# cindytsai/multigrid_poisson_solver

Hardware: AMD Instinct MI355X
Metric: vcycle_mlups (higher is better)
Workload: dtype f64; 1 GPU; V(3,3)-cycle N=8192^2 fp64, 11 levels to N=8, red-black GS(1e-7) coarse solve, cycle-file driver (eager, stream smoother: temporally blocked wave-streaming kernels on the large levels, register-tile kernels on the levels 65..1024, one-workgroup LDS kernel below; halos recomputed, neighbours via DPP lane shifts); N=8192, levels=11

## Files before the change

### include/mg_hip.h

```cpp
#ifndef MG_HIP_H
#define MG_HIP_H

#include <stddef.h>
#include <stdint.h>

#ifdef __cplusplus
extern "C" {
#endif

int         mg_init(int device);
void        mg_finalize(void);
void        mg_set_stream(void *hip_stream);
void       *mg_get_stream(void);
void        mg_sync(void);
int         mg_last_error(void);
const char *mg_last_error_string(void);
void        mg_clear_error(void);
void        mg_set_abort_on_error(int on);
int         mg_set_smoother(const char *name);
const char *mg_version(void);

double *mg_alloc(size_t n_doubles);
void    mg_free(double *dev);
void    mg_pool_trim(void);
// ... 36 lines not shown
void   mg_download_f32(float *host, const float *dev, size_t n);
void mg_prolongAdd(int N, const double *U_c, int M, const double *U_f_in, double *U_f_out);
void mg_restrict_signed(int N, const double *U_f, int M, double *U_c, int sign);
int  mg_lastExactSolverIterations(void);

void mg_restriction_table(int N, int M, int *lo, double *w);
void mg_prolongation_table(int N, int M, int axis, int *owner, double *w_hi, double *w_lo);

void mg_fill_uniform(double *dst, size_t n_doubles, uint64_t seed);
void mg_checksum(const double *src, size_t n_doubles, uint64_t out[2]);

typedef struct mg_profile_entry {
    char   name[64];
    int    N;
    int    launches;
    double total_ms;
    double algo_bytes;
} mg_profile_entry;
void mg_profile_begin(int min_N);
void mg_profile_sample(int every);
int  mg_profile_end(mg_profile_entry *out, int cap);

typedef struct mg_node_record {
    int    node;
    int    N;
    int    steps;
    double error;
} mg_node_record;

typedef struct mg_cycle_result {
    int     status;
    int     N;
    double *U_dev;
    double  mg_error;
    double  time_ms;
    double  device_ms;
    int     n_records;
    const mg_node_record *records;
    const char *report;
    int     graph_replayed;
    int     schedule_launches;
} mg_cycle_result;

typedef struct mg_cycle_plan mg_cycle_plan;

#define MG_CYCLE_FUSED   1
#define MG_CYCLE_GRAPH   2
#define MG_CYCLE_REPORT  4
#define MG_CYCLE_ERROR   8
#define MG_CYCLE_MIXED  16

mg_cycle_plan *mg_cycle_load(const char *path, int flags);
int            mg_cycle_execute(mg_cycle_plan *plan, mg_cycle_result *out);
int            mg_cycle_enqueue(mg_cycle_plan *plan);
int            mg_cycle_collect(mg_cycle_plan *plan, mg_cycle_result *out);
int            mg_cycle_set_refinement(mg_cycle_plan *plan, int cycles);
int            mg_cycle_refinement_errors(mg_cycle_plan *plan, double *out, int cap);
void           mg_cycle_destroy(mg_cycle_plan *plan);
int            mg_cycle_main(int argc, char **argv);
int            mg_print2File(int N, const double *U_dev, const char *file_name);

int  mg_comm_unique_id_bytes(void);
int  mg_comm_get_unique_id(void *out);
int  mg_comm_init(int rank, int nranks, const void *unique_id);
typedef struct mg_host_transport {
    void *user;
    int (*exchange)(void *user, int n_ops, const int *is_send, const int *peer, void *const *buf, const size_t *bytes);
    int (*allgather)(void *user, const double *send, double *recv, size_t count_per_rank);
} mg_host_transport;
int  mg_comm_init_host(int rank, int nranks, const mg_host_transport *transport);
int  mg_comm_selftest(size_t n_doubles);
void mg_comm_finalize(void);
int  mg_comm_rank(void);
int  mg_comm_size(void);
const char *mg_comm_library(void);

int  mg_slab_partition(int N_max, int N_min, int nranks, int collapse_N, int *out, int *collapsed_out);
int  mg_slab_ghost_rows(void);
int  mg_slab_schedule(int N_max, int N_min, int nranks, int collapse_N, int steps, int ca_mode, int ca_pct,
                      int *level_out, int *rank_out);
int  mg_slab_recompute_levels(int N_max, int N_min, int steps, int *pre_out);
int  mg_slab_recompute_levels_ranks(int N_max, int N_min, int steps, int nranks, int *pre_out);
int  mg_recompute_pair_available(int pre, int post);

typedef struct mg_slab_plan mg_slab_plan;
mg_slab_plan *mg_slab_load(const char *path, int nranks, int rank, int collapse_N);
mg_slab_plan *mg_slab_load_flags(const char *path, int nranks, int rank, int collapse_N, int flags);
int  mg_slab_set_refinement(mg_slab_plan *plan, int cycles);
int  mg_slab_refinement_errors(mg_slab_plan *plan, double *out, int cap);
int  mg_slab_execute(mg_slab_plan *plan, mg_cycle_result *out);
int  mg_slab_enqueue(mg_slab_plan *plan);
int  mg_slab_collect(mg_slab_plan *plan, mg_cycle_result *out);
int  mg_slab_gather_U(mg_slab_plan *plan, double *host_full);
void mg_slab_want_error(mg_slab_plan *plan, int on);
void mg_slab_destroy(mg_slab_plan *plan);

typedef struct mg_solve_opts {
    int    pre, post;
    int    N_min;
    double omega;
    double coarse_rtol, coarse_atol;
    int    coarse_max_iters;
    double rtol, atol;
    int    max_cycles;
    double shift;
} mg_solve_opts;

#define MG_SOLVE_CONVERGED      0
#define MG_SOLVE_NOT_CONVERGED (-1)

typedef struct mg_solve_result {
    int    status;
    int    cycles;
    int    converged;
    int    coarse_capped;
    double res0, res, ref_norm;
    double device_ms;
    int    n_history;
    const double *history;
} mg_solve_result;

typedef struct mg_solver mg_solver;

void       mg_solve_opts_default(mg_solve_opts *o);
mg_solver *mg_solver_create(int N, double L, const mg_solve_opts *o);
int        mg_solver_solve(mg_solver *s, const double *F_dev, double *U_dev, mg_solve_result *out);
void       mg_solver_destroy(mg_solver *s);

typedef struct mg_batch_solve_stats {
    int    cycles;
    int    launches;
    double device_ms;
} mg_batch_solve_stats;

typedef struct mg_batch_solver mg_batch_solver;

mg_batch_solver *mg_batch_solver_create(int N, double L, int max_batch, const mg_solve_opts *o);
int  mg_batch_solver_solve(mg_batch_solver *s, int n, const double *const *F_dev, double *const *U_dev, mg_solve_result *out,
                           mg_batch_solve_stats *stats);
void mg_batch_solver_destroy(mg_batch_solver *s);

#ifdef __cplusplus
}
#endif
#endif
```

### multigrid_poisson_solver_amd/__init__.py

```python
import ctypes as C
import importlib.util
import os
import sys

import numpy as np

_PKG = os.path.dirname(os.path.abspath(__file__))
LIB_PATH = os.environ.get("MG_LIB") or os.path.join(_PKG, "lib", "libmgpoisson.so")
EXE_PATH = os.path.join(_PKG, "bin", "MG_HIP")

MG_CYCLE_FUSED, MG_CYCLE_GRAPH, MG_CYCLE_REPORT, MG_CYCLE_ERROR, MG_CYCLE_MIXED = 1, 2, 4, 8, 16


class MGError(RuntimeError):
    pass


class NodeRecord(C.Structure):
    _fields_ = [("node", C.c_int), ("N", C.c_int), ("steps", C.c_int), ("error", C.c_double)]


class ProfileEntry(C.Structure):
    _fields_ = [("name", C.c_char * 64), ("N", C.c_int), ("launches", C.c_int), ("total_ms", C.c_double),
                ("algo_bytes", C.c_double)]


class CycleResult(C.Structure):
    _fields_ = [("status", C.c_int), ("N", C.c_int), ("U_dev", C.c_void_p), ("mg_error", C.c_double),
                ("time_ms", C.c_double), ("device_ms", C.c_double), ("n_records", C.c_int),
                ("records", C.POINTER(NodeRecord)), ("report", C.c_char_p), ("graph_replayed", C.c_int),
                ("schedule_launches", C.c_int)]


_vp, _i, _d, _sz, _u64 = C.c_void_p, C.c_int, C.c_double, C.c_size_t, C.c_uint64
_dptr = C.POINTER(C.c_double)


class SolveOpts(C.Structure):
    _fields_ = [("pre", C.c_int), ("post", C.c_int), ("N_min", C.c_int), ("omega", C.c_double), ("coarse_rtol", C.c_double),
                ("coarse_atol", C.c_double), ("coarse_max_iters", C.c_int), ("rtol", C.c_double), ("atol", C.c_double),
                ("max_cycles", C.c_int), ("shift", C.c_double)]


class SolveResult(C.Structure):
    _fields_ = [("status", C.c_int), ("cycles", C.c_int), ("converged", C.c_int), ("coarse_capped", C.c_int),
                ("res0", C.c_double), ("res", C.c_double), ("ref_norm", C.c_double), ("device_ms", C.c_double),
                ("n_history", C.c_int), ("history", _dptr)]


class BatchSolveStats(C.Structure):
    _fields_ = [("cycles", C.c_int), ("launches", C.c_int), ("device_ms", C.c_double)]


MG_SOLVE_CONVERGED, MG_SOLVE_NOT_CONVERGED = 0, -1

ABI = {
    "mg_init": (_i, [_i]), "mg_finalize": (None, []), "mg_set_stream": (None, [_vp]),
    "mg_get_stream": (_vp, []), "mg_sync": (None, []), "mg_last_error": (_i, []),
    "mg_last_error_string": (C.c_char_p, []), "mg_clear_error": (None, []),
    "mg_set_abort_on_error": (None, [_i]), "mg_set_smoother": (_i, [C.c_char_p]),
    "mg_version": (C.c_char_p, []), "mg_set_source": (_i, [C.c_char_p]), "mg_source_mode": (C.c_char_p, []),
    "mg_source_is_bit_identical": (_i, []),
    "mg_alloc": (_vp, [_sz]), "mg_free": (None, [_vp]), "mg_pool_trim": (None, []),
    "mg_pool_bytes": (_sz, []), "mg_upload": (None, [_vp, _vp, _sz]), "mg_download": (None, [_vp, _vp, _sz]),
    "mg_copy": (None, [_vp, _vp, _sz]), "mg_fill_zero": (None, [_vp, _sz]), "mg_negate": (None, [_i, _vp]),
    "mg_getSource": (None, [_i, _d, _vp, _d, _d]), "mg_getAnalytic": (None, [_i, _d, _vp, _d, _d]),
    "mg_analyticError": (None, [_i, _d, _vp, _d, _d, _dptr]),
    "mg_getResidual": (None, [_i, _d, _vp, _vp, _vp]), "mg_doGridAddition": (None, [_i, _vp, _vp]),
    "mg_doSmoothing": (None, [_i, _d, _vp, _vp, _i, _dptr]),
    "mg_doExactSolver": (None, [_i, _d, _vp, _vp, _d, _i]),
    "mg_doRestriction": (None, [_i, _vp, _i, _vp]), "mg_doProlongation": (None, [_i, _vp, _i, _vp]),
    "mg_smooth_pp": (None, [_i, _d, _vp, _vp, _vp, _i, _vp, _vp, _i]),
    "mg_smooth_restrict": (None, [_i, _d, _vp, _vp, _vp, _i, _vp, _i, _vp]),
    "mg_prolong_smooth": (None, [_i, _vp, _i, _d, _vp, _vp, _vp, _i, _vp]),
    "mg_cycle_set_refinement": (_i, [_vp, _i]), "mg_cycle_refinement_errors": (_i, [_vp, _vp, _i]),
    "mg_smooth_restrict_f32": (None, [_i, _d, _vp, _vp, _vp, _i, _vp, _i, _vp]),
    "mg_prolong_smooth_f32": (None, [_i, _vp, _i, _d, _vp, _vp, _vp, _i, _vp]),
    "mg_alloc_f32": (_vp, [_sz]), "mg_free_f32": (None, [_vp]), "mg_to_f32": (None, [_vp, _vp, _sz]),
    "mg_to_f64": (None, [_vp, _vp, _sz]), "mg_upload_f32": (None, [_vp, _vp, _sz]),
    "mg_download_f32": (None, [_vp, _vp, _sz]),
    "mg_prolongAdd": (None, [_i, _vp, _i, _vp, _vp]), "mg_restrict_signed": (None, [_i, _vp, _i, _vp, _i]),
    "mg_lastExactSolverIterations": (_i, []),
    "mg_restriction_table": (None, [_i, _i, _vp, _vp]),
    "mg_prolongation_table": (None, [_i, _i, _i, _vp, _vp, _vp]),
    "mg_fill_uniform": (None, [_vp, _sz, _u64]), "mg_checksum": (None, [_vp, _sz, C.POINTER(_u64)]),
    "mg_cycle_load": (_vp, [C.c_char_p, _i]), "mg_cycle_execute": (_i, [_vp, C.POINTER(CycleResult)]),
    "mg_cycle_enqueue": (_i, [_vp]), "mg_cycle_collect": (_i, [_vp, C.POINTER(CycleResult)]),
    "mg_cycle_destroy": (None, [_vp]), "mg_cycle_main": (_i, [_i, C.POINTER(C.c_char_p)]),
    "mg_print2File": (_i, [_i, _vp, C.c_char_p]),
    "mg_comm_unique_id_bytes": (_i, []), "mg_comm_get_unique_id": (_i, [_vp]),
    "mg_comm_init_host": (_i, [_i, _i, _vp]),
    "mg_comm_init": (_i, [_i, _i, _vp]), "mg_comm_finalize": (None, []), "mg_comm_selftest": (_i, [_sz]), "mg_comm_rank": (_i, []),
    "mg_comm_size": (_i, []),
    "mg_comm_library": (C.c_char_p, []),
    "mg_slab_partition": (_i, [_i, _i, _i, _i, _vp, _vp]), "mg_slab_ghost_rows": (_i, []),
    "mg_slab_set_refinement": (_i, [_vp, _i]), "mg_slab_refinement_errors": (_i, [_vp, _vp, _i]),
    "mg_slab_schedule": (_i, [_i, _i, _i, _i, _i, _i, _i, _vp, _vp]),
    "mg_slab_recompute_levels": (_i, [_i, _i, _i, _vp]), "mg_slab_recompute_levels_ranks": (_i, [_i, _i, _i, _i, _vp]),
    "mg_recompute_pair_available": (_i, [_i, _i]),
    "mg_slab_load": (_vp, [C.c_char_p, _i, _i, _i]), "mg_slab_load_flags": (_vp, [C.c_char_p, _i, _i, _i, _i]), "mg_slab_execute": (_i, [_vp, C.POINTER(CycleResult)]),
    "mg_slab_enqueue": (_i, [_vp]), "mg_slab_collect": (_i, [_vp, C.POINTER(CycleResult)]),
    "mg_slab_gather_U": (_i, [_vp, _vp]), "mg_slab_want_error": (None, [_vp, _i]), "mg_slab_destroy": (None, [_vp]),
    "mg_solve_opts_default": (None, [C.POINTER(SolveOpts)]),
    "mg_solver_create": (_vp, [_i, _d, C.POINTER(SolveOpts)]),
    "mg_solver_solve": (_i, [_vp, _vp, _vp, C.POINTER(SolveResult)]), "mg_solver_destroy": (None, [_vp]),
    "mg_batch_solver_create": (_vp, [_i, _d, _i, C.POINTER(SolveOpts)]),
    "mg_batch_solver_solve": (_i, [_vp, _i, _vp, _vp, _vp, C.POINTER(BatchSolveStats)]),
    "mg_batch_solver_destroy": (None, [_vp]),
    "mg_profile_begin": (None, [_i]), "mg_profile_sample": (None, [_i]), "mg_profile_end": (_i, [C.POINTER(ProfileEntry), _i]),
}

_lib = None
hip_runtime = None


def _bind_hip_runtime():
    global hip_runtime
    mode = os.environ.get("MG_HIP_RUNTIME", "auto")
    hip_runtime = "system"
    if mode == "system":
        return
    if mode not in ("auto", "torch"):
        C.CDLL(mode, mode=C.RTLD_GLOBAL)
        hip_runtime = mode
        return
    if "torch" in sys.modules:
        hip_runtime = "torch (imported before the engine)"
        return
    try:
        spec = importlib.util.find_spec("torch")
    except (ImportError, ValueError):
        spec = None
    if spec is None or not spec.submodule_search_locations:
        return
    cand = os.path.join(list(spec.submodule_search_locations)[0], "lib", "libamdhip64.so")
    if os.path.exists(cand):
        C.CDLL(cand, mode=C.RTLD_GLOBAL)
        hip_runtime = cand


def load_library(path=None):
    global _lib
    if _lib is not None:
        return _lib
    path = path or LIB_PATH
    if not os.path.exists(path):
        raise MGError(f"{path} is missing: run `python -c 'import __graft_entry__ as g; g.build()'` "
                      "(hipcc, gfx950).  There is no CPU fallback.")
    _bind_hip_runtime()
    lib = C.CDLL(path, mode=C.RTLD_GLOBAL)
    missing = []
    for name, (res, args) in ABI.items():
        try:
            fn = getattr(lib, name)
        except AttributeError:
            missing.append(name)
            continue
        fn.restype, fn.argtypes = res, args
    if missing:
        raise MGError(f"{path} does not export: {missing}")
    _lib = lib
    return lib


def _check():
    code = _lib.mg_last_error()
    if code:
        msg = _lib.mg_last_error_string().decode()
        _lib.mg_clear_error()
        raise MGError(f"[{code}] {msg}")


_initialised = False


def init(device=0):
    global _initialised
    lib = load_library()
    lib.mg_set_abort_on_error(0)
    if lib.mg_init(int(device)) != 0:
        code = lib.mg_last_error()
        msg = lib.mg_last_error_string().decode()
# ... 799 lines not shown
```

### multigrid_poisson_solver_amd/csrc/mg_abi.cpp

```cpp
#include <cmath>
#include <cstdarg>
#include <cstdlib>
#include <cstring>

#include "mg_internal.h"

namespace mg {

Context &ctx()
{
    static Context c;
    return c;
}

void fail(int code, const char *fmt, ...)
{
    char buf[512];
    va_list ap;
    va_start(ap, fmt);
    vsnprintf(buf, sizeof buf, fmt, ap);
    va_end(ap);
    Context &c = ctx();
    c.last_error = code;
    c.last_error_text = buf;
    fprintf(stderr, "[ ERROR ]: %s\n", buf);
    if (c.abort_on_error) exit(1);
}

bool hip_ok(hipError_t e, const char *what, const char *file, int line)
{
    if (e == hipSuccess) return true;
    fail(MG_ERR_HIP, "HIP call failed: %s -> %s (%s:%d)", what, hipGetErrorString(e), file, line);
    return false;
}

bool require_ready(const char *who)
{
    if (ctx().ready) return true;
    fail(MG_ERR_NOT_INIT, "%s: mg_init() has not been called (or failed); there is no CPU fallback", who);
    return false;
}

void *Pool::get(size_t bytes)
{
    if (bytes == 0) bytes = 8;
    bytes = (bytes + 255) & ~(size_t)255;
    auto it = free_.find(bytes);
    if (it != free_.end()) {
        void *p = it->second;
        free_.erase(it);
        live_[p] = bytes;
        if (poison_) poison_block(p, bytes);
        return p;
    }
    void *p = nullptr;
    hipError_t e = hipMalloc(&p, bytes);
    if (e != hipSuccess) {
        (void)hipGetLastError();
        trim();
        if (!MG_HIP(hipMalloc(&p, bytes))) return nullptr;
    }
    held_ += bytes;
    live_[p] = bytes;
    if (poison_) poison_block(p, bytes);
    return p;
}

bool pool_poison_wanted()
{
    const char *e = getenv("MG_POOL_POISON");
    return e && strcmp(e, "0") != 0;
}

void poison_block(void *p, size_t bytes)
{
    if (!p) return;
    hipStream_t s = ctx().stream;
    hipStreamCaptureStatus cs = hipStreamCaptureStatusNone;
    if (hipStreamIsCapturing(s, &cs) != hipSuccess) (void)hipGetLastError();
    if (cs != hipStreamCaptureStatusNone) return;
    (void)MG_HIP(hipMemsetAsync(p, 0xFF, bytes, s));
}

void Pool::put(void *p)
{
    if (!p) return;
    auto it = live_.find(p);
    if (it == live_.end()) {
// ... 1012 lines not shown
}

void mg_restrict_signed(int N, const double *U_f, int M, double *U_c, int sign)
{
    if (!require_ready("doRestriction") || !grid_args_ok("doRestriction", N) || !grid_args_ok("doRestriction", M)) return;
    const RestrictTable &t = restrict_table(N, M);
    if (!t.lo) return;
    ProfScope ps("restrict", N, 8.0 * N * N + 8.0 * M * M);
    k::restrict_gather(ctx().stream, N, U_f, M, U_c, t, sign < 0 ? -1 : +1);
}

void mg_doRestriction(int N, double *U_f, int M, double *U_c) { mg_restrict_signed(N, U_f, M, U_c, +1); }

void mg_doProlongation(int N, double *U_c, int M, double *U_f)
{
    if (!require_ready("doProlongation") || !grid_args_ok("doProlongation", N) || !grid_args_ok("doProlongation", M)) return;
    const ProlongTable &t = prolong_table(N, M);
    if (!t.owner_row) return;
    ProfScope ps("prolong", M, 8.0 * N * N + 8.0 * M * M);
    k::prolong(ctx().stream, N, U_c, M, nullptr, U_f, t);
}

void mg_prolongAdd(int N, const double *U_c, int M, const double *U_f_in, double *U_f_out)
{
    if (!require_ready("mg_prolongAdd") || !grid_args_ok("mg_prolongAdd", N) || !grid_args_ok("mg_prolongAdd", M)) return;
    const ProlongTable &t = prolong_table(N, M);
    if (!t.owner_row) return;
    ProfScope ps("prolong_add", M, 8.0 * N * N + 16.0 * M * M);
    k::prolong(ctx().stream, N, U_c, M, U_f_in, U_f_out, t);
}

void mg_profile_begin(int min_N)
{
    if (!require_ready("mg_profile_begin")) return;
    Context &c = ctx();
    (void)hipStreamSynchronize(c.stream);
    for (auto &r : c.prof) {
        c.event_pool.push_back(r.e0);
        c.event_pool.push_back(r.e1);
    }
    c.prof.clear();
    c.profile_min_N = min_N;
    c.profile_window = 0;
    c.profiling = true;
}

void mg_profile_sample(int every) { ctx().profile_every = every < 1 ? 1 : every; }

int mg_profile_end(mg_profile_entry *out, int cap)
{
    if (!require_ready("mg_profile_end")) return 0;
    Context &c = ctx();
    c.profiling = false;
    (void)hipStreamSynchronize(c.stream);
    int count = 0;
    for (auto &r : c.prof) {
        float ms = 0.f;
        if (hipEventElapsedTime(&ms, r.e0, r.e1) != hipSuccess) {
            (void)hipGetLastError();
            ms = 0.f;
        }
        int j = 0;
        for (; j < count; ++j)
            if (out[j].N == r.N && r.name == out[j].name) break;
        if (j == count) {
            if (count >= cap) continue;
            memset(&out[j], 0, sizeof out[j]);
            snprintf(out[j].name, sizeof out[j].name, "%s", r.name.c_str());
            out[j].N = r.N;
            out[j].algo_bytes = r.bytes;
            ++count;
        }
        out[j].launches += 1;
        out[j].total_ms += ms;
        c.event_pool.push_back(r.e0);
        c.event_pool.push_back(r.e1);
    }
    c.prof.clear();
    return count;
}

int mg_recompute_pair_available(int pre, int post) { return k::stream_recompute_supported(pre, post) ? 1 : 0; }

void mg_restriction_table(int N, int M, int *lo, double *w) { build_restriction_table(N, M, lo, w); }
void mg_prolongation_table(int N, int M, int axis, int *owner, double *w_hi, double *w_lo)
{
    build_prolongation_table(N, M, axis, owner, w_hi, w_lo);
}

void mg_fill_uniform(double *dst, size_t n, uint64_t seed)
{
    if (!require_ready("mg_fill_uniform")) return;
    k::fill_uniform(ctx().stream, dst, n, seed);
}

void mg_checksum(const double *src, size_t n, uint64_t out[2])
{
    if (!require_ready("mg_checksum")) return;
    Context &c = ctx();
    uint64_t *slot = (uint64_t *)(c.scalars + Scalars::CHECKSUM);
    k::checksum(c.stream, src, n, slot);
    if (MG_HIP(hipMemcpyAsync(c.host_scalars, slot, 2 * sizeof(uint64_t), hipMemcpyDeviceToHost, c.stream)) &&
        MG_HIP(hipStreamSynchronize(c.stream))) {
        memcpy(out, c.host_scalars, 2 * sizeof(uint64_t));
    }
}

}
```

### multigrid_poisson_solver_amd/csrc/mg_stream_impl.h

```cpp
#include <hip/hip_runtime.h>

#include <type_traits>
#include <utility>

#include <algorithm>
#include <cstdlib>
#include <vector>

#include "mg_divconst.h"
#include "mg_internal.h"
#include "mg_lane_ops.h"

#if !defined(MG_REAL) || !defined(MG_REAL_NS)
#error "define MG_REAL (double|float) and MG_REAL_NS (f64|f32) before including mg_stream_impl.h"
#endif

namespace mg {
namespace k {
namespace MG_REAL_NS {

typedef MG_REAL real_t;

constexpr int PF_DEFAULT = 2;
#ifndef MG_WAVES_PER_WG
#define MG_WAVES_PER_WG 4
#endif
constexpr int WAVES_PER_WG = MG_WAVES_PER_WG;
constexpr int MAX_S = 4;
#ifndef MG_PF
#define MG_PF 2
#endif

constexpr bool recompute_instantiated(int pre, int steps)
{
    return MG_PF == 2 && pre >= 1 && steps >= 1 && pre <= MAX_S && steps <= MAX_S && pre + steps <= 6;
}

enum InMode { IN_LOAD = 0, IN_ZERO = 1, IN_PROLONG = 2 };

typedef real_t real2_t __attribute__((ext_vector_type(2)));
typedef real_t real4_t __attribute__((ext_vector_type(4)));

struct StreamParams {
    int N;
    real_t dx2, inv;
    const real_t *in;
    const real_t *F;
    real_t *out;
    real_t *D;
    int d_sign;
    double *part;
    long long *trace;
    int cols4;
    int rows_per_chunk;
    int groups;
    int n_blocks;
    int row_base, rows_local, own_y0, own_y1;
    int norm_y0, norm_y1;
    double *out_wide;
    int coarse_base, coarse_rows;
    int raw_norm;
    int nt_min_n;
    int no_out;
    int pre;
    int fc_base, fc_rows;
    const real_t *coarse;
    int Nc;
    const int *p_orow, *p_ocol;
    const real_t *p_rhi, *p_rlo, *p_chi, *p_clo;
    real_t c_dx, c_dx_rcp;
    real_t *Fc;
    int M;
    const int *r_inv;
    const real_t *r_w;
    const real_t *r_wf;
    const NodeBatchItem *batch;
    int part_stride;
    int n_batch;
    double *const *err_outs;
    real_t cw;
    int wt;
    real_t dc;
    int sh;
};


typedef const int __attribute__((address_space(4))) *const_int_ptr;
typedef const real_t __attribute__((address_space(4))) *const_real_ptr;
__device__ __forceinline__ int table_i(const int *t, int i) { return ((const_int_ptr)(uintptr_t)t)[i]; }
__device__ __forceinline__ real_t table_d(const real_t *t, int i) { return ((const_real_ptr)(uintptr_t)t)[i]; }

template <int COLS>
struct Row {
    real_t v[COLS];
};

#ifndef MG_ZERO_LEVEL1
#define MG_ZERO_LEVEL1 1
#endif
#ifndef MG_NT_LOADS
#define MG_NT_LOADS 0
#endif
template <int COLS, bool NT = false>
__device__ __forceinline__ Row<COLS> load_row(const real_t *__restrict__ row, unsigned col_bytes)
{
    Row<COLS> r;
    const char *a = reinterpret_cast<const char *>(row) + col_bytes;
    if constexpr (COLS == 2) {
        const real2_t t = NT ? __builtin_nontemporal_load(reinterpret_cast<const real2_t *>(a)) : *reinterpret_cast<const real2_t *>(a);
        r.v[0] = t.x;
        r.v[1] = t.y;
    } else if constexpr (COLS == 4) {
        const real4_t t = NT ? __builtin_nontemporal_load(reinterpret_cast<const real4_t *>(a)) : *reinterpret_cast<const real4_t *>(a);
        r.v[0] = t.x;
        r.v[1] = t.y;
        r.v[2] = t.z;
        r.v[3] = t.w;
    } else {
        r.v[0] = *reinterpret_cast<const real_t *>(a);
    }
    return r;
}

template <int COLS, bool NT>
__device__ __forceinline__ void store_row(real_t *__restrict__ row, unsigned col_bytes, const Row<COLS> &r)
{
    char *a = reinterpret_cast<char *>(row) + col_bytes;
    if constexpr (COLS == 2) {
        real2_t t;
        t.x = r.v[0];
        t.y = r.v[1];
        if constexpr (NT) __builtin_nontemporal_store(t, reinterpret_cast<real2_t *>(a));
        else *reinterpret_cast<real2_t *>(a) = t;
    } else if constexpr (COLS == 4) {
        real4_t t;
        t.x = r.v[0];
        t.y = r.v[1];
        t.z = r.v[2];
        t.w = r.v[3];
        if constexpr (NT) __builtin_nontemporal_store(t, reinterpret_cast<real4_t *>(a));
        else *reinterpret_cast<real4_t *>(a) = t;
    } else {
        *reinterpret_cast<real_t *>(a) = r.v[0];
    }
}

template <int S, bool RESTRICT, int COLS = 2>
struct Halo {
    static constexpr int A = COLS > 2 ? COLS : 2;
    static constexpr int value = (S + (RESTRICT ? 2 : 1) + A - 1) / A * A;
};


template <int NCV>
struct CoarseV {
    real_t v[NCV];
};
template <int NCV>
__device__ __forceinline__ CoarseV<NCV> load_coarse(const real_t *__restrict__ coarse, int Nc, int base, int rows, int row,
                                                    const unsigned (&col)[NCV])
{
    CoarseV<NCV> c;
    int r = row - base;
    r = r < 0 ? 0 : (r < rows - 1 ? r : rows - 1);
    const char *b = reinterpret_cast<const char *>(coarse + (size_t)r * Nc);
#pragma unroll
    for (int q = 0; q < NCV; ++q) c.v[q] = *reinterpret_cast<const real_t *>(b + col[q]);
    return c;
}


template <int NCV>
__device__ __forceinline__ CoarseV<NCV> load_coarse_local(const real_t *__restrict__ coarse, int Nc, int local_row, const unsigned (&col)[NCV])
{
    CoarseV<NCV> c;
    const char *b = reinterpret_cast<const char *>(coarse + (size_t)local_row * Nc);
#pragma unroll
    for (int q = 0; q < NCV; ++q) c.v[q] = *reinterpret_cast<const real_t *>(b + col[q]);
    return c;
}

template <class F, int... K>
__device__ __forceinline__ void unrolled_while(F &&f, std::integer_sequence<int, K...>)
{
    (void)(f(std::integral_constant<int, K>{}) && ...);
}

#ifndef MG_WPE_DOWN
#define MG_WPE_DOWN 0
#endif
template <int S, int COLS, int IN, bool RESTRICT, int PRE>
struct WavesPerSimd {
    static constexpr int min = (MG_WPE_DOWN > 0 && sizeof(real_t) == 8 && COLS == 2 && IN == 1  && RESTRICT && S <= 3) ? MG_WPE_DOWN : 1;
};

#ifndef MG_LDS_RING
#define MG_LDS_RING 1
#endif
#ifndef MG_PACKED_F32
#define MG_PACKED_F32 1
#endif
typedef float pk_t __attribute__((ext_vector_type(2)));
__device__ __forceinline__ pk_t pk(float a, float b)
{
    pk_t r;
    r.x = a;
    r.y = b;
    return r;
}
__device__ __forceinline__ pk_t pk_fma(pk_t a, pk_t b, pk_t c) { return __builtin_elementwise_fma(a, b, c); }
__device__ __forceinline__ pk_t pk_div_by_const(pk_t x, float c, float rc)
{
    const pk_t cc = pk(c, c), rr = pk(rc, rc);
    pk_t q = x * rr;
    pk_t r = pk_fma(-q, cc, x);
    q = pk_fma(r, rr, q);
    r = pk_fma(-q, cc, x);
    return pk_fma(r, rr, q);
}
template <int COLS, int PRE>
struct LdsRing {
    static constexpr bool value = MG_LDS_RING && PRE > 0 && (COLS == 2 || (COLS == 4 && sizeof(real_t) == 4));
};
template <int COLS> struct RingVec { typedef real_t full; typedef real_t half; };
template <> struct RingVec<2> { typedef real2_t full; typedef real_t half; };
template <> struct RingVec<4> { typedef real4_t full; typedef real2_t half; };
template <int COLS>
__device__ __forceinline__ typename RingVec<COLS>::full ring_pack(const Row<COLS> &r)
{
    typename RingVec<COLS>::full t;
    if constexpr (COLS == 1) t = r.v[0];
    else {
#pragma unroll
        for (int j = 0; j < COLS; ++j) t[j] = r.v[j];
    }
    return t;
}
template <int COLS>
__device__ __forceinline__ Row<COLS> ring_unpack(const typename RingVec<COLS>::full &t)
{
    Row<COLS> r;
    if constexpr (COLS == 1) r.v[0] = t;
    else {
#pragma unroll
        for (int j = 0; j < COLS; ++j) r.v[j] = t[j];
    }
    return r;
}
#ifndef MG_PF_UP
#define MG_PF_UP 3
#endif
#ifndef MG_PF_DOWN
#define MG_PF_DOWN 3
#endif
#ifndef MG_WPE_UP
#define MG_WPE_UP 2
#endif

template <bool SH>
__device__ __forceinline__ real_t minus_centre(real_t a, real_t u, real_t dc)
{
    if constexpr (SH) return a - dc * u;
    else return minus4(a, u);
}

template <int S, int COLS, int IN, bool RESTRICT, int PF = PF_DEFAULT, bool NT = false, int PRE = 0, bool WT = false, bool SH = false>
__global__ __launch_bounds__(64 * WAVES_PER_WG) __attribute__((amdgpu_waves_per_eu(LdsRing<COLS, PRE>::value ? MG_WPE_UP : WavesPerSimd<S, COLS, IN, RESTRICT, PRE>::min)))
void k_jacobi_stream(const StreamParams p)
{
    static_assert(COLS == 2 || COLS == 4 || (IN != IN_PROLONG && !RESTRICT), "fused transfer stages need column pairs");
    static_assert(COLS != 4 || sizeof(real_t) == 4, "4 columns per lane = one 16-byte access: fp32 fields only");
    constexpr int NCV = COLS / 2 + 2;
    constexpr int NS = COLS >= 2 ? COLS / 2 : 1;
    static_assert(PRE == 0 || (IN == IN_PROLONG && !RESTRICT), "recomputed pre-smoothing belongs to the fused `1` node");
    static_assert(!WT || (PRE == 0 && sizeof(real_t) == 8), "the weighted sweep: fp64 nodes that store and re-read U");
    static_assert(!SH || WT, "the screened operator is a form of the weighted sweep");
    constexpr int L = S + PRE;
    constexpr bool LDSR = LdsRing<COLS, PRE>::value;
    constexpr bool HALF = LDSR;
    constexpr bool PACKED = MG_PACKED_F32 && (COLS == 2 || COLS == 4) && sizeof(real_t) == 4;
#ifndef MG_TB_DIRECT
#define MG_TB_DIRECT 0
#endif
    constexpr bool TB_DIRECT = LDSR && MG_TB_DIRECT;
    constexpr int NB = LDSR ? 8 : (PF + L + 2 <= 8 ? 8 : 16);
    constexpr int NFR = LDSR ? (PF < 4 ? 4 : 8) : NB;
    static_assert((LDSR ? L + 2 <= NB : PF + L + 2 <= NB) && PF < 8, "the F ring has NB slots, the U ring 4 or 8");
    static_assert(!LDSR || (IN == IN_PROLONG && !RESTRICT), "the LDS ring belongs to the recomputing `1` node");
    typedef typename RingVec<COLS>::full ring_t;
    typedef typename RingVec<COLS>::half ringh_t;
    __shared__ ring_t s_g[LDSR ? WAVES_PER_WG : 1][LDSR ? NB : 1][LDSR ? 64 : 1];
    __shared__ ringh_t s_f[LDSR ? WAVES_PER_WG : 1][LDSR ? NB : 1][LDSR ? 64 : 1];
    constexpr int W = 64 * COLS;
    constexpr int H = Halo<L, RESTRICT, COLS>::value;
    constexpr int OW = W - 2 * H;

#ifdef MG_STREAM_TRACE
    const long long tr0 = wall_clock64();
#endif
    const int per_xcd = (p.n_blocks + 7) >> 3;
    const int tile = (int)(blockIdx.x & 7) * per_xcd + (int)(blockIdx.x >> 3);
    if (tile >= p.n_blocks) return;
    const real_t *a_in = p.in, *a_F = p.F, *a_coarse = p.coarse;
    real_t *a_out = p.out, *a_Fc = p.Fc;
    double *a_part = p.part;
    if (p.batch) {
        typedef const NodeBatchItem __attribute__((address_space(4))) *item_ptr;
        const item_ptr b = (item_ptr)(uintptr_t)(p.batch + blockIdx.y);
        a_in = static_cast<const real_t *>(b->in);
        a_F = static_cast<const real_t *>(b->F);
        a_coarse = static_cast<const real_t *>(b->coarse);
        a_out = static_cast<real_t *>(b->out);
        a_Fc = static_cast<real_t *>(b->Fc);
        if (a_part) a_part += (size_t)blockIdx.y * (size_t)p.part_stride;
    }
    const int chunk = tile / p.groups;
    const int group = tile - chunk * p.groups;

    const int lane = threadIdx.x & 63;
    const int wave = threadIdx.x >> 6;
    const int strip = group * WAVES_PER_WG + wave;
    const int N = p.N;
    const int own_x0 = strip * OW;
    if (own_x0 >= N) {
        if (a_part && lane == 0) a_part[(size_t)tile * WAVES_PER_WG + wave] = 0.0;
        return;
    }
    const int y0 = p.own_y0 + chunk * p.rows_per_chunk;
    int y1 = y0 + p.rows_per_chunk;
    if (y1 > p.own_y1) y1 = p.own_y1;
    if (y0 >= p.own_y1) return;
    const int av_lo = p.row_base > 0 ? p.row_base : 0;
    const int av_hi = p.row_base + p.rows_local < N ? p.row_base + p.rows_local : N;

    const int xl = own_x0 - H + lane * COLS;
    bool col_in[COLS], col_edge[COLS];
    bool lane_owns = true;
    real_t qc[COLS];
#pragma unroll
    for (int j = 0; j < COLS; ++j) {
        const int x = xl + j;
        col_in[j] = x >= 0 && x < N;
        col_edge[j] = x <= 0 || x >= N - 1;
        lane_owns = lane_owns && x >= own_x0 && x < own_x0 + OW && x < N;
        qc[j] = col_edge[j] ? real_t(0.0) : (WT ? p.cw : real_t(0.25));
    }
    int nm_even[COLS], nm_odd[COLS];
#pragma unroll
    for (int j = 0; j < COLS; ++j) {
        const bool mine = lane_owns && !col_edge[j];
        nm_even[j] = (mine && ((xl + j) & 1) == 0) ? -1 : 0;
        nm_odd[j] = (mine && ((xl + j) & 1) != 0) ? -1 : 0;
    }
    const bool lane_loads = col_in[0] && col_in[COLS - 1];
    const real_t dx2 = p.dx2, inv = p.inv;
    const real_t dc = SH ? p.dc : real_t(4.0);
    const bool want_res = RESTRICT || p.D != nullptr || p.part != nullptr;
    const unsigned col_off = (unsigned)(xl < 0 ? 0 : (xl > N - COLS ? N - COLS : xl)) * (unsigned)sizeof(real_t);
    const unsigned col_st = (unsigned)(xl < 0 ? 0 : xl) * (unsigned)sizeof(real_t);
    const unsigned row_bytes = (unsigned)N * (unsigned)sizeof(real_t);

    unsigned pc_col[NCV];
    int pc_cell[COLS];
    real_t pc_hi[COLS], pc_lo[COLS];
    real_t hA[COLS], hB[COLS];
#pragma unroll
    for (int q = 0; q < NCV; ++q) pc_col[q] = 0u;
#pragma unroll
    for (int j = 0; j < COLS; ++j) {
        pc_cell[j] = 0;
        pc_hi[j] = pc_lo[j] = hA[j] = hB[j] = real_t(0.0);
    }
    int c_row = -0x40000000;
    if constexpr (IN == IN_PROLONG) {
        if (lane_loads) {
            const int pc_base = p.p_ocol[xl];
            const int last = p.Nc - 1;
#pragma unroll
            for (int j = 0; j < COLS; ++j) {
                pc_cell[j] = p.p_ocol[xl + j] - pc_base;
                pc_hi[j] = p.p_chi[xl + j];
                pc_lo[j] = p.p_clo[xl + j];
            }
#pragma unroll
            for (int q = 0; q < NCV; ++q) pc_col[q] = (unsigned)(pc_base + q < last ? pc_base + q : last) * (unsigned)sizeof(real_t);
        }
    }
    auto interpolate = [&](const CoarseV<NCV> &c, real_t (&h)[COLS]) {
#pragma unroll
        for (int j = 0; j < COLS; ++j) {
            real_t ca = c.v[0], cb = c.v[1];
#pragma unroll
            for (int q = 1; q + 1 < NCV; ++q) {
                const bool here = pc_cell[j] == q;
                ca = here ? c.v[q] : ca;
                cb = here ? c.v[q + 1] : cb;
            }
            h[j] = ca * pc_hi[j] + cb * pc_lo[j];
        }
    };

    int rc_col[NS];
    bool rc_shift[NS];
    real_t rw_a[NS], rw_b[NS];
    Row<COLS> d_prev;
#pragma unroll
    for (int j = 0; j < COLS; ++j) d_prev.v[j] = 0.0;
#pragma unroll
    for (int q = 0; q < NS; ++q) {
        rc_col[q] = -1;
        rc_shift[q] = false;
        rw_a[q] = rw_b[q] = real_t(0.0);
    }
    if constexpr (RESTRICT) {
        if (lane_owns) {
#pragma unroll
            for (int q = 0; q < NS; ++q) {
                const int ca = p.r_inv[xl + 2 * q], cb = p.r_inv[xl + 2 * q + 1];
                rc_col[q] = ca >= 0 ? ca : cb;
                rc_shift[q] = ca < 0 && cb >= 0;
                if (rc_col[q] >= 0) {
                    rw_a[q] = p.r_w[rc_col[q]];
                    rw_b[q] = real_t(1.0) - rw_a[q];
                }
            }
        }
    }
// ... 377 lines not shown
                    const real_t r = inv * minus_centre<SH>(nw.v[j] + so.v[j] + e + w, c.v[j], dc) - f.v[j];
                    if constexpr (RESTRICT) {
                        d.v[j] = r * hi_bits_and(ms[j], inner);
                    } else {
                        d.v[j] = r;
                    }
                    if constexpr (EVEN_START) {
                        if ((j & 1) == (k & 1)) acc += fabs(bits_and((double)r, ((lane_owns && !col_edge[j]) ? -1 : 0) & cm));
                    } else {
                        const int am = ((k & 1) ? nm_k1[j] : nm_k0[j]) & cm;
                        acc += fabs(bits_and((double)r, am));
                    }
                }
                if constexpr (!RESTRICT) {
                    if (mine_row && lane_owns && p.D) {
                        Row<COLS> ds;
#pragma unroll
                        for (int j = 0; j < COLS; ++j) {
                            const real_t dv = (inner != 0 && !col_edge[j]) ? d.v[j] : real_t(0.0);
                            ds.v[j] = p.d_sign < 0 ? -dv : dv;
                        }
                        store_row<COLS, false>(reinterpret_cast<real_t *>(reinterpret_cast<char *>(p.D) + (st_off - (long long)row_bytes)), col_st, ds);
                    }
                } else {
                    if (mine_row && lane_owns && p.D)
                        store_row<COLS, false>(reinterpret_cast<real_t *>(reinterpret_cast<char *>(p.D) + (st_off - (long long)row_bytes)), col_st, d);
                }

                if constexpr (RESTRICT) {
                    const int rc_row = lane_value(tb_rc, t & 63);
                    if (rc_row >= 0) {
                        const real_t wc = lane_value(tb_rw, t & 63), wd = real_t(1.0) - wc;
                        const real_t p_up = from_lane_above(d_prev.v[0]);
                        const real_t q_up = from_lane_above(d.v[0]);
                        real_t *crow = a_Fc + (size_t)(rc_row - p.fc_base) * p.M;
#pragma unroll
                        for (int q = 0; q < NS; ++q) {
                            const real_t p_next = q + 1 < NS ? d_prev.v[q + 1 < NS ? 2 * q + 2 : 0] : p_up;
                            const real_t q_next = q + 1 < NS ? d.v[q + 1 < NS ? 2 * q + 2 : 0] : q_up;
                            const real_t u0 = rc_shift[q] ? d_prev.v[2 * q + 1] : d_prev.v[2 * q];
                            const real_t u1 = rc_shift[q] ? p_next : d_prev.v[2 * q + 1];
                            const real_t u2 = rc_shift[q] ? d.v[2 * q + 1] : d.v[2 * q];
                            const real_t u3 = rc_shift[q] ? q_next : d.v[2 * q + 1];
                            const real_t vc = rw_b[q] * wd * u0 + rw_a[q] * wd * u1 + wc * rw_b[q] * u2 + rw_a[q] * wc * u3;
                            if (rc_col[q] >= 0) crow[rc_col[q]] = vc;
                        }
                        if (first_col_lane) crow[0] = 0.0;
                        if (last_col_lane) crow[p.M - 1] = 0.0;
                    }
                    d_prev = d;
                }
            }
            older[L] = newer[L];
            newer[L] = nw;
            st_off += row_bytes;
            return true;
        };
        unrolled_while(row_step, std::make_integer_sequence<int, NB>{});
    }
#ifdef MG_STREAM_TRACE
    if (p.trace && (threadIdx.x & 63) == 0) {
        const long long tr2 = wall_clock64();
        long long *rec = p.trace + 8 + 4 * ((size_t)tile * WAVES_PER_WG + wave);
        rec[0] = tr0;
        rec[1] = tr1;
        rec[2] = tr2;
        rec[3] = (long long)blockIdx.x;
        if (tile == p.n_blocks / 2 && wave == 0) {
            p.trace[0] = tr0;
            p.trace[1] = tr1;
            p.trace[2] = tr2;
            p.trace[3] = T;
        }
    }
#endif
    if (a_part) {
#pragma unroll
        for (int o = 32; o > 0; o >>= 1) acc += __shfl_down(acc, o, 64);
        if (lane == 0) a_part[(size_t)tile * WAVES_PER_WG + wave] = acc;
    }
}

#ifndef MG_STREAM_KERNEL_ONLY
template <int S, int COLS, int IN, bool RESTRICT, int PF = PF_DEFAULT, bool NT = false, int PRE = 0, bool WT = false, bool SH = false>
void launch_k(hipStream_t s, StreamParams p, double *err_out)
{
    static int blocks_per_cu = 0;
    if (blocks_per_cu == 0) {
        int n = 0;
        if (hipOccupancyMaxActiveBlocksPerMultiprocessor(&n, k_jacobi_stream<S, COLS, IN, RESTRICT, PF, NT, PRE, WT, SH>, 64 * WAVES_PER_WG, 0) != hipSuccess || n < 1) {
            (void)hipGetLastError();
            n = 2;
        }
        blocks_per_cu = n > 8 ? 8 : n;
    }
    const int N = p.N;
    const int own = p.own_y1 - p.own_y0;
    if (own <= 0) return;
    constexpr int OW = 64 * COLS - 2 * Halo<S + PRE, RESTRICT, COLS>::value;
    const int strips = (N + OW - 1) / OW;
    const int groups = (strips + WAVES_PER_WG - 1) / WAVES_PER_WG;
    static const int resident_pct = [] { const char *e = getenv("MG_RESIDENT_PCT"); return e ? atoi(e) : 100; }();
    const int resident = ctx().n_cu * blocks_per_cu * resident_pct / 100;
    const int nb = p.batch ? p.n_batch : 1;
    int chunks = resident / (groups * nb);
    static const int min_rows_forced = [] { const char *e = getenv("MG_MIN_ROWS"); return e ? atoi(e) : 0; }();
    const int min_rows = min_rows_forced ? min_rows_forced : (N <= 256 ? 2 : N <= 1024 ? 4 : 8);
    const int max_chunks = (own + min_rows - 1) / min_rows;
    if (chunks > max_chunks) chunks = max_chunks;
    if (chunks < 1) chunks = 1;
    int rows = (own + chunks - 1) / chunks;
    static const int rows_cap = [] { const char *e = getenv("MG_MAX_ROWS"); return e ? atoi(e) : 0; }();
    if (rows_cap > 0 && rows > rows_cap) rows = rows_cap;
    if (LdsRing<COLS, PRE>::value) {
        const int march = rows + 2 * (S + PRE + 1);
        rows += (8 - march % 8) % 8;
    } else if (COLS >= 2) {
        rows += rows & 1;
    }
    chunks = (own + rows - 1) / rows;
    p.rows_per_chunk = rows;
    p.groups = groups;
    p.n_blocks = chunks * groups;
    p.part = nullptr;
#ifdef MG_STREAM_TRACE
    static long long *trace_dev = nullptr;
    if (!trace_dev) (void)hipMalloc((void **)&trace_dev, (8 + 4 * 4 * 4096) * sizeof(long long));
    (void)hipMemsetAsync(trace_dev, 0, (8 + 4 * 4 * 4096) * sizeof(long long), s);
    p.trace = trace_dev;
#endif
    const size_t n_part = (size_t)p.n_blocks * WAVES_PER_WG;
    const bool want_norm = err_out || (p.batch && p.err_outs);
    if (want_norm) {
        p.part = norm_partials(n_part * (size_t)nb);
        if (!p.part) return;
    }
    p.part_stride = (int)n_part;
    const int grid = ((p.n_blocks + 7) / 8) * 8;
    hipLaunchKernelGGL((k_jacobi_stream<S, COLS, IN, RESTRICT, PF, NT, PRE, WT, SH>), dim3(grid, nb), dim3(64 * WAVES_PER_WG), 0, s, p);
#ifdef MG_STREAM_TRACE
    {
        long long t[4];
        (void)hipStreamSynchronize(s);
        (void)hipMemcpy(t, trace_dev, sizeof t, hipMemcpyDeviceToHost);
        fprintf(stderr, "[stream trace] N=%d IN=%d R=%d tiles=%d rows/chunk=%d: prologue %.2f us, %lld steps %.2f us (%.3f us/step)\n", N, IN, (int)RESTRICT,
                p.n_blocks, rows, (t[1] - t[0]) * 0.01, t[3], (t[2] - t[1]) * 0.01, (t[2] - t[1]) * 0.01 / (double)t[3]);
        if (N >= 4096 && p.n_blocks <= 4096) {
            const size_t nw = (size_t)p.n_blocks * WAVES_PER_WG;
            std::vector<long long> all(4 * nw);
            (void)hipMemcpy(all.data(), trace_dev + 8, all.size() * sizeof(long long), hipMemcpyDeviceToHost);
            long long t_min = 0x7fffffffffffffffll, t_max = 0;
            std::vector<double> start, life, endt;
            for (size_t w = 0; w < nw; ++w) {
                if (all[4 * w] == 0) continue;
                if (all[4 * w] < t_min) t_min = all[4 * w];
                if (all[4 * w + 2] > t_max) t_max = all[4 * w + 2];
            }
            double xcd_end[8] = {0}, xcd_start[8] = {0};
            for (size_t w = 0; w < nw; ++w) {
                if (all[4 * w] == 0) continue;
                start.push_back((all[4 * w] - t_min) * 0.01);
                endt.push_back((all[4 * w + 2] - t_min) * 0.01);
                life.push_back((all[4 * w + 2] - all[4 * w]) * 0.01);
                const int x = (int)(all[4 * w + 3] & 7);
                if (endt.back() > xcd_end[x]) xcd_end[x] = endt.back();
                if (start.back() > xcd_start[x]) xcd_start[x] = start.back();
            }
            auto pct = [](std::vector<double> v, double q) { std::sort(v.begin(), v.end()); return v[(size_t)(q * (v.size() - 1))]; };
            fprintf(stderr, "   waves %zu: start p50 %.1f p99 %.1f max %.1f us | lifetime p1 %.1f p50 %.1f p99 %.1f max %.1f | end p1 %.1f p50 %.1f p99 %.1f max %.1f | span %.1f us\n",
                    nw, pct(start, .5), pct(start, .99), pct(start, 1.0), pct(life, .01), pct(life, .5), pct(life, .99), pct(life, 1.0), pct(endt, .01),
                    pct(endt, .5), pct(endt, .99), pct(endt, 1.0), (t_max - t_min) * 0.01);
            fprintf(stderr, "   last wave per XCD ends at:");
            for (int x = 0; x < 8; ++x) fprintf(stderr, " %.1f", xcd_end[x]);
            fprintf(stderr, " us\n");
        }
    }
#endif
    if (p.batch && p.err_outs) {
        for (int i = 0; i < nb; ++i)
            if (p.err_outs[i]) norm_finish(s, p.part + (size_t)i * n_part, n_part, p.raw_norm ? -1 : N, p.err_outs[i]);
    } else if (err_out) {
        norm_finish(s, p.part, n_part, p.raw_norm ? -1 : N, err_out);
    }
}

template <int S, int PF>
void launch_variant(hipStream_t s, const StreamParams &p, double *err_out)
{
    const bool restrict_out = p.Fc != nullptr, prolong_in = p.coarse != nullptr, zero = p.in == nullptr;
    const bool nt = p.N >= p.nt_min_n;
    if constexpr (sizeof(real_t) == 4) {
        if (p.cols4 && !(prolong_in && p.pre)) {
            if (restrict_out) {
                if (zero) launch_k<S, 4, IN_ZERO, true, PF>(s, p, err_out);
                else launch_k<S, 4, IN_LOAD, true, PF>(s, p, err_out);
            } else if (prolong_in) {
                if (nt) launch_k<S, 4, IN_PROLONG, false, PF, true>(s, p, err_out);
                else launch_k<S, 4, IN_PROLONG, false, PF>(s, p, err_out);
            } else {
                if (zero) launch_k<S, 4, IN_ZERO, false, PF>(s, p, err_out);
                else launch_k<S, 4, IN_LOAD, false, PF>(s, p, err_out);
            }
            return;
        }
    }
    if constexpr (sizeof(real_t) == 8) {
        if (p.wt) {
            auto weighted = [&](auto sh_tag) {
                constexpr bool SH = decltype(sh_tag)::value;
                if (p.N % 2 != 0) {
                    if (zero) launch_k<S, 1, IN_ZERO, false, PF, false, 0, true, SH>(s, p, err_out);
                    else launch_k<S, 1, IN_LOAD, false, PF, false, 0, true, SH>(s, p, err_out);
                } else if (restrict_out) {
                    if (zero) launch_k<S, 2, IN_ZERO, true, (PF == 2 && S <= 3 ? MG_PF_DOWN : PF), false, 0, true, SH>(s, p, err_out);
                    else launch_k<S, 2, IN_LOAD, true, PF, false, 0, true, SH>(s, p, err_out);
                } else if (prolong_in) {
                    if (p.pre != 0) fail(MG_ERR_UNSUPPORTED, "jacobi_stream: no recomputing `1` node for the weighted sweep");
                    else if (nt) launch_k<S, 2, IN_PROLONG, false, PF, true, 0, true, SH>(s, p, err_out);
                    else launch_k<S, 2, IN_PROLONG, false, PF, false, 0, true, SH>(s, p, err_out);
                } else {
                    if (zero) launch_k<S, 2, IN_ZERO, false, PF, false, 0, true, SH>(s, p, err_out);
                    else launch_k<S, 2, IN_LOAD, false, PF, false, 0, true, SH>(s, p, err_out);
                }
            };
            if (p.sh) weighted(std::true_type{});
            else weighted(std::false_type{});
            return;
        }
    }
// ... 144 lines not shown
```

Before: 788,400 MLUPS.

## Flatten stream kernel tiling to per-wave strips with edge-aligned windows

Replaces the per-workgroup strip grouping with a flat wave-level decomposition. Waves are packed across chunks so no workgroup slots go idle for strips past the domain edge. Windows are aligned to the domain edge so the first and last strips waste fewer halo lanes, and the chunk count is computed from wave slots rather than group slots. It also caps waves-per-EU at 3 for the S=3 restrict-fused f64 kernel and adds host geometry query/logging helpers. The legacy tiling is kept behind an environment variable.

```diff
diff --git a/include/mg_hip.h b/include/mg_hip.h
--- a/include/mg_hip.h
+++ b/include/mg_hip.h
@@ -142,6 +142,8 @@
 int  mg_slab_recompute_levels(int N_max, int N_min, int steps, int *pre_out);
 int  mg_slab_recompute_levels_ranks(int N_max, int N_min, int steps, int nranks, int *pre_out);
 int  mg_recompute_pair_available(int pre, int post);
+int  mg_stream_geometry(const int *args, int *out);
+int  mg_stream_wave_tile(const int *args, int w, int *out);
 
 typedef struct mg_slab_plan mg_slab_plan;
 mg_slab_plan *mg_slab_load(const char *path, int nranks, int rank, int collapse_N);
diff --git a/multigrid_poisson_solver_amd/__init__.py b/multigrid_poisson_solver_amd/__init__.py
--- a/multigrid_poisson_solver_amd/__init__.py
+++ b/multigrid_poisson_solver_amd/__init__.py
@@ -98,6 +98,7 @@
     "mg_slab_schedule": (_i, [_i, _i, _i, _i, _i, _i, _i, _vp, _vp]),
     "mg_slab_recompute_levels": (_i, [_i, _i, _i, _vp]), "mg_slab_recompute_levels_ranks": (_i, [_i, _i, _i, _i, _vp]),
     "mg_recompute_pair_available": (_i, [_i, _i]),
+    "mg_stream_geometry": (_i, [_vp, _vp]), "mg_stream_wave_tile": (_i, [_vp, _i, _vp]),
     "mg_slab_load": (_vp, [C.c_char_p, _i, _i, _i]), "mg_slab_load_flags": (_vp, [C.c_char_p, _i, _i, _i, _i]), "mg_slab_execute": (_i, [_vp, C.POINTER(CycleResult)]),
     "mg_slab_enqueue": (_i, [_vp]), "mg_slab_collect": (_i, [_vp, C.POINTER(CycleResult)]),
     "mg_slab_gather_U": (_i, [_vp, _vp]), "mg_slab_want_error": (None, [_vp, _i]), "mg_slab_destroy": (None, [_vp]),
diff --git a/multigrid_poisson_solver_amd/csrc/mg_abi.cpp b/multigrid_poisson_solver_amd/csrc/mg_abi.cpp
--- a/multigrid_poisson_solver_amd/csrc/mg_abi.cpp
+++ b/multigrid_poisson_solver_amd/csrc/mg_abi.cpp
@@ -4,6 +4,7 @@
 #include <cstring>
 
 #include "mg_internal.h"
+#include "mg_stream_geom.h"
 
 namespace mg {
 
@@ -1182,6 +1183,30 @@
 
 int mg_recompute_pair_available(int pre, int post) { return k::stream_recompute_supported(pre, post) ? 1 : 0; }
 
+static k::StreamGeom geom_of(const int *a)
+{
+    return k::stream_geometry(a[0], a[1], a[2], a[3], a[4], a[5], a[6] != 0, a[7], a[8], a[9], a[10] != 0, a[11] != 0);
+}
+int mg_stream_geometry(const int *args, int *out)
+{
+    if (!args || !out) return -1;
+    const k::StreamGeom g = geom_of(args);
+    if (g.strips < 1) return -1;
+    const int v[10] = {g.strips, g.strip_slots, g.win_shift, g.ow, g.chunks, g.rows, g.march, g.waves, g.workgroups, MG_WAVES_PER_WG};
+    memcpy(out, v, sizeof v);
+    return 0;
+}
+int mg_stream_wave_tile(const int *args, int w, int *out)
+{
+    if (!args || !out || w < 0) return -1;
+    const k::StreamGeom g = geom_of(args);
+    if (g.strips < 1) return -1;
+    const k::WaveTile t = k::stream_wave_tile(g, w);
+    const int v[6] = {t.active, t.chunk, t.strip, t.win_x0, t.own_lo, t.own_hi};
+    memcpy(out, v, sizeof v);
+    return 0;
+}
+
 void mg_restriction_table(int N, int M, int *lo, double *w) { build_restriction_table(N, M, lo, w); }
 void mg_prolongation_table(int N, int M, int axis, int *owner, double *w_hi, double *w_lo)
 {
diff --git a/multigrid_poisson_solver_amd/csrc/mg_stream_geom.h b/multigrid_poisson_solver_amd/csrc/mg_stream_geom.h
--- /dev/null
+++ b/multigrid_poisson_solver_amd/csrc/mg_stream_geom.h
@@ -0,0 +1,96 @@
+#pragma once
+
+#if defined(__HIP__) || defined(__CUDACC__)
+#define MG_GEOM_HD __host__ __device__
+#else
+#define MG_GEOM_HD
+#endif
+
+#ifndef MG_WAVES_PER_WG
+#define MG_WAVES_PER_WG 4
+#endif
+
+namespace mg {
+namespace k {
+
+struct StreamGeom {
+    int legacy;
+    int N, H, W, ow;
+    int strips;
+    int strip_slots;
+    int win_shift;
+    int chunks, rows;
+    int march;
+    int waves;
+    int workgroups;
+};
+
+struct WaveTile {
+    int active, chunk, strip;
+    int win_x0;
+    int own_lo, own_hi;
+};
+
+MG_GEOM_HD inline WaveTile stream_wave_tile(int w, int waves, int strip_slots, int last_strip, int win_shift, int N, int H, int W)
+{
+    WaveTile t;
+    t.chunk = w / strip_slots;
+    t.strip = w - t.chunk * strip_slots;
+    t.active = (w < waves && t.strip <= last_strip) ? 1 : 0;
+    t.win_x0 = t.strip * (W - 2 * H) - win_shift;
+    t.own_lo = t.strip == 0 ? 0 : t.win_x0 + H;
+    t.own_hi = t.strip == last_strip ? N : t.win_x0 + W - H;
+    return t;
+}
+
+inline StreamGeom stream_geometry(int N, int own_rows, int H, int W, int slots, int n_batch, bool lds_ring, int march_extra, int min_rows,
+                                  int max_rows, bool even_rows, bool legacy)
+{
+    constexpr int WPW = MG_WAVES_PER_WG;
+    StreamGeom g = {};
+    g.legacy = legacy ? 1 : 0;
+    g.N = N;
+    g.H = H;
+    g.W = W;
+    g.ow = W - 2 * H;
+    if (N < 1 || own_rows < 1 || H < 0 || g.ow < 1) return g;
+    if (n_batch < 1) n_batch = 1;
+    if (min_rows < 1) min_rows = 1;
+    int chunks;
+    if (legacy) {
+        g.strips = (N + g.ow - 1) / g.ow;
+        const int groups = (g.strips + WPW - 1) / WPW;
+        g.strip_slots = groups * WPW;
+        g.win_shift = H;
+        chunks = (slots / WPW) / (groups * n_batch);
+    } else {
+        g.strips = N <= W ? 1 : 1 + (N - W + g.ow - 1) / g.ow;
+        g.strip_slots = g.strips;
+        g.win_shift = 0;
+        chunks = slots / (g.strips * n_batch);
+    }
+    const int max_chunks = (own_rows + min_rows - 1) / min_rows;
+    if (chunks > max_chunks) chunks = max_chunks;
+    if (chunks < 1) chunks = 1;
+    int rows = (own_rows + chunks - 1) / chunks;
+    if (max_rows > 0 && rows > max_rows) rows = max_rows;
+    if (lds_ring) {
+        rows += (8 - (rows + march_extra) % 8) % 8;
+    } else if (even_rows) {
+        rows += rows & 1;
+    }
+    g.rows = rows;
+    g.chunks = (own_rows + rows - 1) / rows;
+    g.march = rows + march_extra;
+    g.waves = g.chunks * g.strip_slots;
+    g.workgroups = (g.waves + WPW - 1) / WPW;
+    return g;
+}
+
+inline WaveTile stream_wave_tile(const StreamGeom &g, int w)
+{
+    return stream_wave_tile(w, g.waves, g.strip_slots, g.strips - 1, g.win_shift, g.N, g.H, g.W);
+}
+
+}
+}
diff --git a/multigrid_poisson_solver_amd/csrc/mg_stream_impl.h b/multigrid_poisson_solver_amd/csrc/mg_stream_impl.h
--- a/multigrid_poisson_solver_amd/csrc/mg_stream_impl.h
+++ b/multigrid_poisson_solver_amd/csrc/mg_stream_impl.h
@@ -5,11 +5,13 @@
 
 #include <algorithm>
 #include <cstdlib>
+#include <cstring>
 #include <vector>
 
 #include "mg_divconst.h"
 #include "mg_internal.h"
 #include "mg_lane_ops.h"
+#include "mg_stream_geom.h"
 
 #if !defined(MG_REAL) || !defined(MG_REAL_NS)
 #error "define MG_REAL (double|float) and MG_REAL_NS (f64|f32) before including mg_stream_impl.h"
@@ -22,9 +24,6 @@
 typedef MG_REAL real_t;
 
 constexpr int PF_DEFAULT = 2;
-#ifndef MG_WAVES_PER_WG
-#define MG_WAVES_PER_WG 4
-#endif
 constexpr int WAVES_PER_WG = MG_WAVES_PER_WG;
 constexpr int MAX_S = 4;
 #ifndef MG_PF
@@ -53,7 +52,8 @@
     long long *trace;
     int cols4;
     int rows_per_chunk;
-    int groups;
+    int strip_slots, last_strip, win_shift;
+    int n_waves;
     int n_blocks;
     int row_base, rows_local, own_y0, own_y1;
     int norm_y0, norm_y1;
@@ -192,6 +192,7 @@
 template <int S, int COLS, int IN, bool RESTRICT, int PRE>
 struct WavesPerSimd {
     static constexpr int min = (MG_WPE_DOWN > 0 && sizeof(real_t) == 8 && COLS == 2 && IN == 1  && RESTRICT && S <= 3) ? MG_WPE_DOWN : 1;
+    static constexpr int max = (MG_WPE_DOWN == 0 && sizeof(real_t) == 8 && COLS == 2 && IN == 1  && RESTRICT && S == 3) ? 3 : 0;
 };
 
 #ifndef MG_LDS_RING
@@ -265,7 +266,7 @@
 }
 
 template <int S, int COLS, int IN, bool RESTRICT, int PF = PF_DEFAULT, bool NT = false, int PRE = 0, bool WT = false, bool SH = false>
-__global__ __launch_bounds__(64 * WAVES_PER_WG) __attribute__((amdgpu_waves_per_eu(LdsRing<COLS, PRE>::value ? MG_WPE_UP : WavesPerSimd<S, COLS, IN, RESTRICT, PRE>::min)))
+__global__ __launch_bounds__(64 * WAVES_PER_WG) __attribute__((amdgpu_waves_per_eu(LdsRing<COLS, PRE>::value ? MG_WPE_UP : WavesPerSimd<S, COLS, IN, RESTRICT, PRE>::min, LdsRing<COLS, PRE>::value ? 0 : WavesPerSimd<S, COLS, IN, RESTRICT, PRE>::max)))
 void k_jacobi_stream(const StreamParams p)
 {
     static_assert(COLS == 2 || COLS == 4 || (IN != IN_PROLONG && !RESTRICT), "fused transfer stages need column pairs");
@@ -293,7 +294,6 @@
     __shared__ ringh_t s_f[LDSR ? WAVES_PER_WG : 1][LDSR ? NB : 1][LDSR ? 64 : 1];
     constexpr int W = 64 * COLS;
     constexpr int H = Halo<L, RESTRICT, COLS>::value;
-    constexpr int OW = W - 2 * H;
 
 #ifdef MG_STREAM_TRACE
     const long long tr0 = wall_clock64();
@@ -314,26 +314,22 @@
         a_Fc = static_cast<real_t *>(b->Fc);
         if (a_part) a_part += (size_t)blockIdx.y * (size_t)p.part_stride;
     }
-    const int chunk = tile / p.groups;
-    const int group = tile - chunk * p.groups;
-
     const int lane = threadIdx.x & 63;
-    const int wave = threadIdx.x >> 6;
-    const int strip = group * WAVES_PER_WG + wave;
+    const int wave = __builtin_amdgcn_readfirstlane((int)(threadIdx.x >> 6));
     const int N = p.N;
-    const int own_x0 = strip * OW;
-    if (own_x0 >= N) {
-        if (a_part && lane == 0) a_part[(size_t)tile * WAVES_PER_WG + wave] = 0.0;
-        return;
-    }
+    const WaveTile wt = stream_wave_tile(tile * WAVES_PER_WG + wave, p.n_waves, p.strip_slots, p.last_strip, p.win_shift, N, H, W);
+    const int chunk = wt.chunk;
     const int y0 = p.own_y0 + chunk * p.rows_per_chunk;
     int y1 = y0 + p.rows_per_chunk;
     if (y1 > p.own_y1) y1 = p.own_y1;
-    if (y0 >= p.own_y1) return;
+    if (!wt.active || y0 >= p.own_y1) {
+        if (a_part && lane == 0) a_part[(size_t)tile * WAVES_PER_WG + wave] = 0.0;
+        return;
+    }
     const int av_lo = p.row_base > 0 ? p.row_base : 0;
     const int av_hi = p.row_base + p.rows_local < N ? p.row_base + p.rows_local : N;
 
-    const int xl = own_x0 - H + lane * COLS;
+    const int xl = wt.win_x0 + lane * COLS;
     bool col_in[COLS], col_edge[COLS];
     bool lane_owns = true;
     real_t qc[COLS];
@@ -342,7 +338,7 @@
         const int x = xl + j;
         col_in[j] = x >= 0 && x < N;
         col_edge[j] = x <= 0 || x >= N - 1;
-        lane_owns = lane_owns && x >= own_x0 && x < own_x0 + OW && x < N;
+        lane_owns = lane_owns && x >= wt.own_lo && x < wt.own_hi;
         qc[j] = col_edge[j] ? real_t(0.0) : (WT ? p.cw : real_t(0.25));
     }
     int nm_even[COLS], nm_odd[COLS];
@@ -886,6 +882,12 @@
 }
 
 #ifndef MG_STREAM_KERNEL_ONLY
+inline bool legacy_tiling()
+{
+    static const bool legacy = [] { const char *e = getenv("MG_STREAM_TILING"); return e && strcmp(e, "legacy") == 0; }();
+    return legacy;
+}
+
 template <int S, int COLS, int IN, bool RESTRICT, int PF = PF_DEFAULT, bool NT = false, int PRE = 0, bool WT = false, bool SH = false>
 void launch_k(hipStream_t s, StreamParams p, double *err_out)
 {
@@ -901,31 +903,32 @@
     const int N = p.N;
     const int own = p.own_y1 - p.own_y0;
     if (own <= 0) return;
-    constexpr int OW = 64 * COLS - 2 * Halo<S + PRE, RESTRICT, COLS>::value;
-    const int strips = (N + OW - 1) / OW;
-    const int groups = (strips + WAVES_PER_WG - 1) / WAVES_PER_WG;
+    constexpr int L = S + PRE, H = Halo<L, RESTRICT, COLS>::value;
     static const int resident_pct = [] { const char *e = getenv("MG_RESIDENT_PCT"); return e ? atoi(e) : 100; }();
     const int resident = ctx().n_cu * blocks_per_cu * resident_pct / 100;
     const int nb = p.batch ? p.n_batch : 1;
-    int chunks = resident / (groups * nb);
     static const int min_rows_forced = [] { const char *e = getenv("MG_MIN_ROWS"); return e ? atoi(e) : 0; }();
     const int min_rows = min_rows_forced ? min_rows_forced : (N <= 256 ? 2 : N <= 1024 ? 4 : 8);
-    const int max_chunks = (own + min_rows - 1) / min_rows;
-    if (chunks > max_chunks) chunks = max_chunks;
-    if (chunks < 1) chunks = 1;
-    int rows = (own + chunks - 1) / chunks;
     static const int rows_cap = [] { const char *e = getenv("MG_MAX_ROWS"); return e ? atoi(e) : 0; }();
-    if (rows_cap > 0 && rows > rows_cap) rows = rows_cap;
-    if (LdsRing<COLS, PRE>::value) {
-        const int march = rows + 2 * (S + PRE + 1);
-        rows += (8 - march % 8) % 8;
-    } else if (COLS >= 2) {
-        rows += rows & 1;
-    }
-    chunks = (own + rows - 1) / rows;
-    p.rows_per_chunk = rows;
-    p.groups = groups;
-    p.n_blocks = chunks * groups;
+    const StreamGeom g = stream_geometry(N, own, H, 64 * COLS, resident * WAVES_PER_WG, nb, LdsRing<COLS, PRE>::value,
+                                         2 * (L + 1) + (RESTRICT ? 1 : 0), min_rows, rows_cap, COLS >= 2, legacy_tiling());
+    p.rows_per_chunk = g.rows;
+    p.strip_slots = g.strip_slots;
+    p.last_strip = g.strips - 1;
+    p.win_shift = g.win_shift;
+    p.n_waves = g.waves;
+    p.n_blocks = g.workgroups;
+    static const bool log_tiling = [] { const char *e = getenv("MG_STREAM_TILING_LOG"); return e && atoi(e) != 0; }();
+    if (log_tiling) {
+        static std::vector<long long> seen;
+        const long long key = ((long long)N << 32) | ((long long)own << 8) | nb;
+        if (std::find(seen.begin(), seen.end(), key) == seen.end()) {
+            seen.push_back(key);
+            fprintf(stderr, "[stream tiling] %s S=%d COLS=%d IN=%d R=%d PRE=%d %s N=%d own=%d batch=%d: wg/CU %d slots %d | H %d strips %d chunks %d rows %d march %d waves %d workgroups %d\n",
+                    g.legacy ? "legacy" : "flat", S, COLS, IN, (int)RESTRICT, PRE, sizeof(real_t) == 8 ? "f64" : "f32", N, own, nb, blocks_per_cu,
+                    resident * WAVES_PER_WG, H, g.strips, g.chunks, g.rows, g.march, g.waves * nb, g.workgroups * nb);
+        }
+    }
     p.part = nullptr;
 #ifdef MG_STREAM_TRACE
     static long long *trace_dev = nullptr;
@@ -948,7 +951,7 @@
         (void)hipStreamSynchronize(s);
         (void)hipMemcpy(t, trace_dev, sizeof t, hipMemcpyDeviceToHost);
         fprintf(stderr, "[stream trace] N=%d IN=%d R=%d tiles=%d rows/chunk=%d: prologue %.2f us, %lld steps %.2f us (%.3f us/step)\n", N, IN, (int)RESTRICT,
-                p.n_blocks, rows, (t[1] - t[0]) * 0.01, t[3], (t[2] - t[1]) * 0.01, (t[2] - t[1]) * 0.01 / (double)t[3]);
+                p.n_blocks, p.rows_per_chunk, (t[1] - t[0]) * 0.01, t[3], (t[2] - t[1]) * 0.01, (t[2] - t[1]) * 0.01 / (double)t[3]);
         if (N >= 4096 && p.n_blocks <= 4096) {
             const size_t nw = (size_t)p.n_blocks * WAVES_PER_WG;
             std::vector<long long> all(4 * nw);
```

New measurement: 782,800 MLUPS. No clear change (-0.7%).
